# sunkafei/coffeedb

Measured on AMD Instinct MI355X. Metric: sa_build_GiB_per_s, higher is better.
Workload: dtype u64

## Files before the change

### coffeedb_amd/csrc/capi.hip

```cpp
#include <dirent.h>

#include <algorithm>
#include <chrono>
#include <condition_variable>
#include <cstdlib>
#include <cstring>
#include <thread>

#include "../../include/coffeedb_gpu.h"
#include "index_impl.h"

using namespace cdb;

namespace {

double wall_ms() {
    using namespace std::chrono;
    return duration<double, std::milli>(steady_clock::now().time_since_epoch()).count();
}

void set_error(Index& ix, const char* msg) {
    std::lock_guard<std::mutex> g(ix.err_mu);
    ix.err = msg;
}
// ... 1553 lines not shown
    else if (!std::strcmp(name, "pack_sa")) ix.pack_sa = value != 0;
    else if (!std::strcmp(name, "key_cost_model")) ix.key_cost_model = value != 0;
    else if (!std::strcmp(name, "gen_prebased")) ix.gen_prebased = value != 0;
    else if (!std::strcmp(name, "pack_entries")) ix.pack_entries = value != 0;
    else if (!std::strcmp(name, "segmented_sort")) ix.segmented_sort = value != 0;
    else if (!std::strcmp(name, "fold_root")) ix.fold_root = value != 0;
    else if (!std::strcmp(name, "fold_depth1")) ix.fold_depth1 = value != 0;
    else if (!std::strcmp(name, "flags_in_last_pass")) ix.flags_in_last_pass = value != 0;
    else if (!std::strcmp(name, "search_lanes")) ix.search_lanes = (value == 1 || value == 8) ? (int)value : 0;
    else if (!std::strcmp(name, "digit_bits")) ix.digit_bits = (int)value;
    else if (!std::strcmp(name, "fuse_keygen")) ix.fuse_keygen = value != 0;
    else if (!std::strcmp(name, "force_big_path")) ix.force_big_path = value != 0;
    else if (!std::strcmp(name, "debug_fail_build")) ix.debug_fail_build = value != 0;
    else if (!std::strcmp(name, "debug_no_segcap")) ix.debug_no_segcap = value != 0;
    else if (!std::strcmp(name, "debug_starve_group")) ix.debug_starve_group = (int)value;
    else if (!std::strcmp(name, "self_check")) ix.self_check = value < 0 ? 0 : value > 3 ? 3 : (int)value;
    else if (!std::strcmp(name, "premap_generation")) ix.premap_generation = value != 0;
    else if (!std::strcmp(name, "proof_cancel")) {
        if (value) proof_stop(ix);
    }
    else if (!std::strcmp(name, "debug_damage_after_build")) ix.debug_damage_after_build = value < 0 ? 0 : (uint64_t)value;
    else if (!std::strcmp(name, "debug_fail_self_check")) ix.debug_fail_self_check = value != 0;
    else if (!std::strcmp(name, "plain_tile_order")) ix.rws.plain_order = value != 0;
    else if (!std::strcmp(name, "key_coding")) ix.key_coding = (int)value;
    else if (!std::strcmp(name, "narrow_keys")) ix.narrow_keys = value != 0;
    else if (!std::strcmp(name, "single_query")) ix.use_single_query = value != 0;
    else if (!std::strcmp(name, "resident_query")) {
        std::lock_guard<std::mutex> g(ix.mu);
        if (value != 1) query_resident_stop(ix);
        ix.resident_mode = value <= 0 ? 0 : value == 1 ? 1 : 2;
        ix.resident_query = ix.resident_mode == 1;
        ix.single_streak = 0;
    }
    else if (!std::strcmp(name, "bucket_group_limit")) ix.bucket_group_limit = (uint64_t)value;
    else if (!std::strcmp(name, "query_hit_budget"))
        ix.query_hit_budget = value > 0 ? std::min<uint64_t>((uint64_t)value, 1ull << 31) : 1;
    else if (!std::strcmp(name, "coalesce_queries")) ix.coalesce_queries = value != 0;
    else if (!std::strcmp(name, "fast_search")) ix.use_fast_search = value != 0;
    else if (!std::strcmp(name, "wave_rows")) ix.use_wave_rows = value != 0;
    else if (!std::strcmp(name, "keep_keys")) ix.keep_keys = value != 0;
    else {
        set_error(ix, (std::string("unknown option: ") + name).c_str());
        return CDB_E_INVALID;
    }
    return CDB_OK;
}

int cdb_get_stat(const cdb_index* h, const char* name, double* value) {
    if (!h || !name || !value) return CDB_E_INVALID;
    const BuildStats& b = h->ix.bstats;
    const QueryStats& q = h->ix.qstats;
    struct { const char* n; double v; } tab[] = {
        {"build_ms", b.build_ms}, {"alloc_ms", b.alloc_ms}, {"free_ms", b.free_ms}, {"rounds", (double)b.rounds}, {"ext_rounds", (double)b.ext_rounds},
        {"dbl_rounds", (double)b.dbl_rounds}, {"unresolved_after_initial", (double)b.unresolved_initial},
        {"unresolved_max", (double)b.unresolved_max}, {"sort_passes", (double)b.sort_passes},
        {"sort_passes_skipped", (double)b.sort_passes_skipped}, {"isa_built", (double)b.isa_built}, {"fused_keygen", (double)b.fused_keygen}, {"dense_keys", (double)b.dense_keys}, {"key_layout", (double)b.key_layout}, {"bucketed", (double)b.bucketed}, {"bucket_groups", (double)b.bucket_groups}, {"segmented", (double)b.segmented}, {"fused_records", (double)b.fused_records}, {"sweep_records", (double)b.sweep_records}, {"vl_key_bits", (double)b.vl_key_bits}, {"partial_levels", (double)b.partial_levels}, {"list_rounds", (double)b.list_rounds}, {"pairclass_fused", (double)b.pairclass_fused}, {"group_sorts", (double)b.group_sorts}, {"group_sort_fallbacks", (double)b.group_sort_fallbacks}, {"vl_avg_len", b.vl_avg_len}, {"vl_rate", b.vl_rate}, {"vl_est_unresolved", b.vl_est_unresolved}, {"fixed_est_unresolved", b.fixed_est_unresolved}, {"gen_prebased", (double)b.gen_prebased}, {"root_folded", (double)b.root_folded}, {"flags_in_last_pass", (double)b.flags_in_last_pass}, {"msd_first", (double)b.msd_first}, {"bucket_low_digits", (double)b.bucket_low_digits}, {"key_directory_cells", h->ix.h_keydir.empty() ? 0.0 : (double)(h->ix.h_keydir.size() - 1)}, {"group_fallbacks", (double)h->ix.group_fallbacks}, {"dense_key_retries", (double)h->ix.dense_key_retries}, {"self_check_fallbacks", (double)h->ix.self_check_fallbacks}, {"sa_packed", h->ix.sa_packed ? 1.0 : 0.0}, {"sa_bytes_per_entry", h->ix.sa_packed ? 5.0 : (double)h->ix.width}, {"self_check_pairs", (double)h->ix.self_check_pairs}, {"self_check_ms", h->ix.self_check_ms}, {"self_check_coverage", h->ix.size > 1 ? (double)h->ix.self_check_pairs / (double)(h->ix.size - 1) : 0.0},
        {"order_proved", (h->ix.proof.state.load() == 2 || h->ix.proof.state.load() == 3 || (h->ix.self_check == 2 && h->ix.width != 0)) ? 1.0 : 0.0},
        {"proof_state", (double)h->ix.proof.state.load()}, {"proof_ms", h->ix.proof.ms}, {"proof_repair_ms", h->ix.proof.repair_ms},
        {"proof_pairs", (double)h->ix.proof.pairs}, {"proof_bad_pairs", (double)h->ix.proof.found[0]}, {"proof_invalid_entries", (double)h->ix.proof.found[1]}, {"proof_skipped_pairs", (double)h->ix.proof.skipped}, {"proof_mixed_pairs", (double)h->ix.proof.mixed},
        {"proof_runs", (double)h->ix.proof.runs}, {"pool_big_mallocs", (double)DevPool::get().big_mallocs()}, {"premap_ms", h->ix.proof.premap_ms}, {"premap_bytes", (double)h->ix.proof.premap_bytes},
        {"key_symbols", (double)b.key_symbols}, {"symbol_bits", (double)b.symbol_bits},
        {"alphabet", (double)b.alphabet}, {"digit_bits", (double)b.digit_bits}, {"final_depth", (double)b.final_depth}, {"compat_rotations", (double)b.compat_rotations},
        {"compat_depth", (double)b.compat_depth},
        {"host_upload_ms", h->ix.host_upload_ms}, {"host_free_ms", h->ix.host_free_ms},
        {"resident_answers", (double)h->ix.res_answers}, {"launched_answers", (double)h->ix.launched_answers}, {"resident_mode", (double)h->ix.resident_mode},
        {"query_ms", q.query_ms}, {"query_upload_ms", q.upload_ms}, {"query_device_ms", q.device_ms}, {"query_download_ms", q.download_ms}, {"query_hits", (double)q.nhits}, {"query_rows", (double)q.nrows},
    };
    for (auto& e : tab)
        if (!std::strcmp(e.n, name)) {
            *value = e.v;
            return CDB_OK;
        }
    return CDB_E_INVALID;
}

int cdb_profile_get(cdb_index* h, const char* kernel, double* total_ms, uint64_t* launches, uint64_t* bytes) {
    if (!h || !kernel) return CDB_E_INVALID;
    std::lock_guard<std::mutex> g(h->ix.mu);
    auto it = h->ix.prof.recs.find(kernel);
    if (it == h->ix.prof.recs.end()) return CDB_E_INVALID;
    if (total_ms) *total_ms = it->second.ms;
    if (launches) *launches = it->second.launches;
    if (bytes) *bytes = it->second.bytes;
    return CDB_OK;
}

int cdb_profile_dump(cdb_index* h, char* buf, size_t cap) {
    if (!h || !buf || cap == 0) return CDB_E_INVALID;
    std::lock_guard<std::mutex> g(h->ix.mu);
// ... 172 lines not shown
```

### coffeedb_amd/csrc/index_impl.h

```cpp
#pragma once
#include <atomic>
#include <condition_variable>
#include <mutex>
#include <thread>
#include <string>
#include <vector>

#include "common.h"
#include "radix_sort.h"

namespace cdb {

constexpr int TEXT_PAD = 128;

struct BuildStats {
    double build_ms = 0, alloc_ms = 0, free_ms = 0;
    int rounds = 0;
    int ext_rounds = 0;
    int dbl_rounds = 0;
    uint64_t unresolved_initial = 0;
    uint64_t unresolved_max = 0;
    int sort_passes = 0;
    int sort_passes_skipped = 0;
    int isa_built = 0;
    int fused_keygen = 0;
    int key_layout = 0;
    int dense_keys = 0;
    int bucketed = 0;
    int bucket_low_digits = 0;
    int bucket_groups = 0;
    int root_folded = 0;
    int flags_in_last_pass = 0;
    int msd_first = 0;
    int gen_prebased = 0;
    int fused_records = 0;
    int sweep_records = 0;
    int pairclass_fused = 0;
    int list_rounds = 0;
    int group_sorts = 0, group_sort_fallbacks = 0;
    int partial_levels = 0;
    int vl_key_bits = 0;
    double vl_avg_len = 0, vl_rate = 0, vl_est_unresolved = 0, fixed_est_unresolved = 0;
    int segmented = 0;
    uint64_t gather_items = 0;
    int key_symbols = 0, symbol_bits = 0, alphabet = 0, digit_bits = 8;
    uint64_t final_depth = 0;
    uint64_t compat_rotations = 0, compat_depth = 0;
};

struct QueryStats {
    double query_ms = 0;
    double upload_ms = 0, device_ms = 0, download_ms = 0;
    uint64_t nhits = 0, nrows = 0;
};

struct SingleKeys {
    const uint64_t* keys64 = nullptr;
    const uint32_t* keys32 = nullptr;
    const void* keylow = nullptr;
    int low_bits = 0, low_bytes = 0, nsym = 0;
    bool decisive = false;
    uint64_t klo = 0, khi = 0;
    bool ranged = false;
    uint64_t lo0 = 0, hi0 = 0;
};

struct Sa40 {
    const uint32_t* __restrict__ lo;
    const uint8_t* __restrict__ hi;
    __device__ __forceinline__ uint64_t operator[](uint64_t i) const { return (uint64_t)lo[i] | ((uint64_t)hi[i] << 32); }
};
struct Packed40 {};
template <typename T> struct SaOf {
    using val = T;
    using ptr = const T* __restrict__;
};
// ... 106 lines not shown

    RadixWorkspace rws;
    MsdWorkspace msd_ws;
    DevBuf scan_partials;
    uint64_t q_spec_cap = 0;
    DevBuf q_spec;
    DevBuf q_pat, q_offs, q_left, q_right, q_hoff, q_keys0, q_keys1, q_flags, q_rowptr, q_ids, q_counts, q_hitptr, q_hitoff;

    bool reference_compat = true;
    bool force_doubling = false;
    int initial_passes = 0;
    int key_symbols = 0;
    int sort_variant = 0;
    int search_lanes = 0;
    bool flags_in_last_pass = true;
    bool fold_depth1 = true;
    bool fold_root = true;
    bool segmented_sort = true;
    bool fuse_records = true;
    bool fuse_pairclass = true;
    bool list_rounds = true;
    int group_sort_cap = 4096;
    bool group_sort = true;
    bool partial_symbol = true;
    int vl_keys = 2;
    bool vl_off_once = false;
    bool sweep_records = true;
    bool pack_entries = true;
    bool msd_first = true;
    bool msd_pair = true;
    bool keyhist3 = true;
    int dense_key_retries = 0;
    int group_fallbacks = 0;
    uint64_t bucket_group_limit = 0;
    uint64_t self_check_pairs = 0;
    double self_check_ms = 0;
    int self_check = 3;
    int self_check_fallbacks = 0;
    bool debug_fail_self_check = false;
    struct Proof {
        std::thread th;
        std::atomic<int> state{0};
        std::atomic<bool> cancel{false};
        hipStream_t stream = nullptr;
        void* d_out = nullptr;
        double ms = 0, repair_ms = 0;
        uint64_t pairs = 0;
        uint64_t found[2] = {0, 0};
        uint64_t skipped = 0;
        uint64_t mixed = 0;
        uint64_t runs = 0;
        bool of_loaded_file = false;
        std::atomic<bool> busy{false};
        bool want_proof = false;
        double premap_ms = 0;
        uint64_t premap_bytes = 0;
    } proof;
    bool premap_generation = false;
    bool proof_in_repair = false;
    uint64_t debug_damage_after_build = 0;
    bool debug_no_segcap = false;
    int debug_starve_group = 0;
    bool debug_fail_build = false;
    bool force_big_path = false;
    bool fuse_keygen = true;
    int digit_bits = 0;
// ... 91 lines not shown
```

### coffeedb_amd/csrc/radix_sort.h

```cpp
#pragma once
#include <cstdlib>

#include "common.h"

namespace cdb {

constexpr int RS_MAX_PASSES = 16;

constexpr uint64_t RS_VAL_MASK = (1ull << 54) - 1;
constexpr uint32_t RS_SPIN_LIMIT_GROUPED = 1u << 18;
constexpr uint32_t RS_SPIN_LIMIT_PLAIN = 1u << 22;
constexpr int RS_GROUP = 8;

struct NoVal {};

template <typename K, typename V> struct RsTraits { static constexpr int IPT = 12; };
template <> struct RsTraits<uint64_t, uint32_t> { static constexpr int IPT = 15; };
template <> struct RsTraits<uint64_t, uint64_t> { static constexpr int IPT = 12; };

template <typename K>
__global__ __launch_bounds__(256) void rs_hist_kernel(const K* __restrict__ keys, uint64_t n, int begin_bit,
                                                      int npass, int dbits, uint32_t last_mask,
                                                      unsigned long long* __restrict__ ghist) {
    __shared__ uint32_t sh[RS_MAX_PASSES * 256];
// ... 1188 lines not shown
        if (need > status.bytes) {
            status.alloc(need + need / 4);
            CDB_HIP(hipMemsetAsync(status.p, 0, status.bytes, s));
            CDB_HIP(hipMemsetAsync(tickets.p, 0, 256 * sizeof(uint32_t), s));
            CDB_HIP(hipMemsetAsync(tickets.as<uint32_t>() + 260, 0, 256 * 8 * sizeof(uint32_t), s));
            epoch = 0;
        }
    }
    uint32_t next_epoch(hipStream_t s) {
        if (epoch == 255) {
            CDB_HIP(hipMemsetAsync(status.p, 0, status.bytes, s));
            CDB_HIP(hipMemsetAsync(tickets.p, 0, 256 * sizeof(uint32_t), s));
            CDB_HIP(hipMemsetAsync(tickets.as<uint32_t>() + 260, 0, 256 * 8 * sizeof(uint32_t), s));
            epoch = 0;
        }
        return ++epoch;
    }
    uint32_t* ticket_ptr(uint32_t e) { return tickets.as<uint32_t>() + (e & 255u); }
    uint32_t* xticket_ptr(uint32_t e) { return tickets.as<uint32_t>() + 260 + (e & 255u) * 8; }
    uint32_t* err_ptr() { return tickets.as<uint32_t>() + 256; }
    void release() { hist.release(); status.release(); tickets.release(); tile_doc.release(); seg1.release(); epoch = 0; }
};

template <typename K, typename V> inline const char* rs_kernel_name();
template <> inline const char* rs_kernel_name<uint64_t, uint32_t>() { return "rs_onesweep_k64_v32"; }
template <> inline const char* rs_kernel_name<uint64_t, uint64_t>() { return "rs_onesweep_k64_v64"; }
template <> inline const char* rs_kernel_name<uint64_t, NoVal>() { return "rs_onesweep_k64"; }
template <> inline const char* rs_kernel_name<uint32_t, uint32_t>() { return "rs_onesweep_k32_v32"; }
template <> inline const char* rs_kernel_name<uint32_t, uint64_t>() { return "rs_onesweep_k32_v64"; }
template <> inline const char* rs_kernel_name<uint32_t, NoVal>() { return "rs_onesweep_k32"; }

struct SortStats {
    int passes_run = 0, passes_skipped = 0;
};

inline bool rs_variant_has_gen(int v) {
    return v == 0 || v == 21 || v == 26 || v == 1 || v == 31 || v == 33 || v == 36 || v == 32;
}

struct SortPlan {
    int npass, begin_bit;
    uint32_t last_mask;
    std::vector<uint64_t> h_hist;
};

template <typename K, typename V, typename Cfg, typename Gen = NoGen, typename W = NoVal>
int radix_sort_cfg(hipStream_t s, RadixWorkspace& ws, Profiler& prof, K* k0, K* k1, V* v0, V* v1, uint64_t n,
                   int begin_bit, int end_bit, SortStats* stats, int dbits, const uint64_t* h_hist_in = nullptr,
                   const Gen* gen = nullptr, W* w0 = nullptr, W* w1 = nullptr, int lead_in = 0,
                   const unsigned long long* d_hist_in = nullptr, const SegFinalKeepArgs* keep = nullptr) {
    constexpr int IPT = Cfg::IPT;
    constexpr int TILE = Cfg::NT * IPT;
    constexpr bool HAS_V = !std::is_same<V, NoVal>::value;
    constexpr bool HAS_W = !std::is_same<W, NoVal>::value;
    constexpr bool GEN = !std::is_same<Gen, NoGen>::value;
    if (dbits < 1 || dbits > 8) dbits = 8;
    int lead = 0;
    if constexpr (GEN && HAS_W) lead = gen->low_bits / dbits;
    else if constexpr (HAS_W) lead = lead_in;
    if (HAS_W && !GEN && !h_hist_in && !d_hist_in) throw Error("radix_sort: split records need caller-supplied histograms (internal)");
    const int LEAD = lead;
    if (n == 0 || end_bit < begin_bit || (!LEAD && end_bit == begin_bit)) return 0;
    const int nbits = end_bit - begin_bit;
    const int kpass = (int)ceil_div(nbits, dbits);
    const int npass = kpass + LEAD;
    if (npass > RS_MAX_PASSES) throw Error("radix_sort: too many passes requested");
// ... 300 lines not shown
        const unsigned long long* dstart = d_starts + (size_t)p * 256;
        uint32_t* tk = grouped ? ws.xticket_ptr(e) : ws.ticket_ptr(e);
        int t = prof.begin(s);
#define CDB_SEG_LAUNCH(CFG, SEGT, SEGV)                                                                                       \
    hipLaunchKernelGGL((rs_onesweep_kernel<uint32_t, uint32_t, CFG, NoGen, W, SEGT>), dim3(grid), dim3(1024), 0, s,            \
                       (const uint32_t*)kb[cur], kb[cur ^ 1], (const uint32_t*)vb[cur], vb[cur ^ 1], m, shift, dmask, dstart, \
                       ws.status.as<uint64_t>(), tk, e, ws.err_ptr(), NoGen(), (const W*)wb[cur], wb[cur ^ 1], aux_shift,     \
                       SEGV)
        if (p == npass - 1) {
            if (grouped) CDB_SEG_LAUNCH(CfgG, SegFinalArgs, fin);
            else CDB_SEG_LAUNCH(CfgP, SegFinalArgs, fin);
            prof.end(t, (std::string("rs_seg_final") + wn + "_t16384").c_str(), m * (rec + (fin.elo ? 6 : 9)), s);
        } else {
            if (grouped) CDB_SEG_LAUNCH(CfgG, SegArgs, sa);
            else CDB_SEG_LAUNCH(CfgP, SegArgs, sa);
            prof.end(t, (std::string("rs_seg_k32_v32") + wn + "_t16384").c_str(), 2 * m * rec, s);
        }
#undef CDB_SEG_LAUNCH
        cur ^= 1;
        if (stats) stats->passes_run++;
    }
    int t = prof.begin(s);
    hipLaunchKernelGGL(rs_seg_edge_fix_kernel, dim3(tiles), dim3(256), 0, s, (const SegEdge*)fin.edges, d_tile_seg, d_segs, tiles,
                       fin.flags, fin.kbase, fin.kmagic, (unsigned long long*)nullptr, 1u, (const uint32_t*)ws.err_ptr());
    prof.end(t, "rs_seg_edge_fix", (uint64_t)tiles * 256 * sizeof(SegEdge), s);
    CDB_HIP(hipGetLastError());
}

constexpr int RS_MSD_HIST_TILES = 32;

template <typename W>
__global__ __launch_bounds__(1024) void rs_seg_hist_kernel(const uint32_t* __restrict__ keys, const W* __restrict__ aux, int lead, int npass,
                                                           const uint32_t* __restrict__ tile_seg, const SegInfo* __restrict__ segs,
                                                           uint32_t tiles, unsigned long long* __restrict__ hist) {
    constexpr int NC = 4, HC = 8 * 256 + 64 / NC;
    __shared__ uint32_t sh4[NC * HC];
    const int tid = threadIdx.x;
    uint32_t* const sh = sh4 + (tid & (NC - 1)) * HC;
    const uint32_t t0 = blockIdx.x * RS_MSD_HIST_TILES;
    const uint32_t t1 = t0 + RS_MSD_HIST_TILES < tiles ? t0 + RS_MSD_HIST_TILES : tiles;
    uint32_t cur = ~0u;
    auto flush = [&]() {
        __syncthreads();
        if (cur != ~0u)
            for (int i = tid; i < npass * 256; i += 1024) {
                uint32_t c = 0;
#pragma unroll
                for (int q = 0; q < NC; ++q) c += sh4[q * HC + i];
                if (c) atomicAdd(&hist[((size_t)cur * 8 + i / 256) * 256 + i % 256], (unsigned long long)c);
            }
        __syncthreads();
        for (int i = tid; i < NC * HC; i += 1024) sh4[i] = 0;
        __syncthreads();
    };
    for (uint32_t t = t0; t < t1; ++t) {
        const uint32_t g = tile_seg[t];
        if (g != cur) {
            flush();
            cur = g;
        }
        const SegInfo si = segs[g];
        const uint64_t base = si.begin + (uint64_t)(t - si.tile_begin) * RS_SEG_TILE;
        const uint32_t valid = (uint32_t)((si.end - base) < (uint64_t)RS_SEG_TILE ? (si.end - base) : (uint64_t)RS_SEG_TILE);
        auto count = [&](uint32_t k, uint32_t a) {
#pragma unroll
            for (int p = 0; p < 8; ++p) {
                if (p < npass) {
                    const uint32_t dg = p < lead ? (a >> (8 * p)) & 0xFFu : (k >> (8 * (p - lead))) & 0xFFu;
                    atomicAdd(&sh[p * 256 + dg], 1u);
                }
            }
        };
        const uint64_t end = base + valid;
        const uint64_t a0 = (base + 3) & ~3ull;
        const uint64_t q0 = a0 < end ? a0 : end;
        const uint32_t nquad = (uint32_t)((end - q0) / 4);
        if ((uint64_t)tid < q0 - base) count(keys[base + tid], lead > 0 ? (uint32_t)aux[base + tid] : 0u);
        {
            const uint64_t tb = q0 + 4ull * nquad;
            if ((uint64_t)tid < end - tb) count(keys[tb + tid], lead > 0 ? (uint32_t)aux[tb + tid] : 0u);
        }
        constexpr int QPT = RS_SEG_TILE / 4 / 1024;
        uint4 kq[QPT];
        uint32_t aq[QPT][4];
#pragma unroll
        for (int r = 0; r < QPT; ++r) {
            const uint32_t g = (uint32_t)r * 1024u + (uint32_t)tid;
            kq[r] = make_uint4(0, 0, 0, 0);
            aq[r][0] = aq[r][1] = aq[r][2] = aq[r][3] = 0;
            if (g < nquad) {
                kq[r] = *reinterpret_cast<const uint4*>(keys + q0 + 4ull * g);
                if (lead > 0) {
                    if constexpr (sizeof(W) == 4) {
                        const uint4 w = *reinterpret_cast<const uint4*>(aux + q0 + 4ull * g);
                        aq[r][0] = w.x; aq[r][1] = w.y; aq[r][2] = w.z; aq[r][3] = w.w;
                    } else if constexpr (sizeof(W) == 2) {
                        const uint2 w = *reinterpret_cast<const uint2*>(aux + q0 + 4ull * g);
                        aq[r][0] = w.x & 0xFFFFu; aq[r][1] = w.x >> 16; aq[r][2] = w.y & 0xFFFFu; aq[r][3] = w.y >> 16;
                    } else {
                        const uint32_t w = *reinterpret_cast<const uint32_t*>(aux + q0 + 4ull * g);
                        aq[r][0] = w & 0xFFu; aq[r][1] = (w >> 8) & 0xFFu; aq[r][2] = (w >> 16) & 0xFFu; aq[r][3] = w >> 24;
                    }
                }
            }
        }
#pragma unroll
        for (int r = 0; r < QPT; ++r) {
            const uint32_t g = (uint32_t)r * 1024u + (uint32_t)tid;
            if (g < nquad) {
                count(kq[r].x, aq[r][0]);
                count(kq[r].y, aq[r][1]);
                count(kq[r].z, aq[r][2]);
                count(kq[r].w, aq[r][3]);
            }
        }
    }
    flush();
}

constexpr int RS_GEN8_TILE = 8192;
constexpr uint32_t RS_TB_ROWS = 256;
static __global__ __launch_bounds__(256) void rs_tilecol_sum_kernel(const uint32_t* __restrict__ counts, uint32_t rows, const uint16_t* __restrict__ src_col,
                                                                    unsigned long long* __restrict__ partial) {
    const uint32_t d = threadIdx.x, b = blockIdx.x;
    const uint32_t c = src_col ? (uint32_t)src_col[d] : d;
    const uint32_t r0 = b * RS_TB_ROWS, r1 = r0 + RS_TB_ROWS < rows ? r0 + RS_TB_ROWS : rows;
    unsigned long long sum = 0;
    if (c < 256u)
        for (uint32_t r = r0; r < r1; ++r) sum += counts[(size_t)r * 256 + c];
    partial[(size_t)b * 256 + d] = sum;
}
static __global__ __launch_bounds__(1024) void rs_tilecol_total_kernel(const unsigned long long* __restrict__ partial, uint32_t blocks,
                                                                       unsigned long long* __restrict__ totals) {
    __shared__ unsigned long long s_q[4][256];
    const uint32_t d = threadIdx.x & 255u, g = threadIdx.x >> 8;
    const uint32_t per = (blocks + 3u) / 4u;
    const uint32_t b0 = g * per, b1 = b0 + per < blocks ? b0 + per : blocks;
    unsigned long long sum = 0;
    uint32_t b = b0;
    for (; b + 8 <= b1; b += 8) {
        unsigned long long v[8];
#pragma unroll
        for (int i = 0; i < 8; ++i) v[i] = partial[(size_t)(b + i) * 256 + d];
#pragma unroll
        for (int i = 0; i < 8; ++i) sum += v[i];
    }
    for (; b < b1; ++b) sum += partial[(size_t)b * 256 + d];
    s_q[g][d] = sum;
    __syncthreads();
    if (g == 0) totals[d] = s_q[0][d] + s_q[1][d] + s_q[2][d] + s_q[3][d];
// ... 308 lines not shown
```

### coffeedb_amd/csrc/sa_build.hip

```cpp
#include <algorithm>
#include <chrono>
#include <cmath>
#include <cstdlib>
#include <cstring>

#include "index_impl.h"
#include "records_sweep.h"
#include "vl_code.h"
#include "scan.h"

#ifndef RS_GATHER_ABL
#define RS_GATHER_ABL 0
#endif

namespace cdb {
namespace {

constexpr int KG_TILE = 2048;
constexpr int KG_LOOK = 64;

__global__ __launch_bounds__(256) void sa_bytecount_kernel(const uint8_t* __restrict__ text, uint64_t n,
                                                           unsigned long long* __restrict__ counts) {
    __shared__ uint32_t s[256];
    s[threadIdx.x] = 0;
// ... 2686 lines not shown
                        constexpr unsigned gather_wgs = 256u * 8u;
                        if (pack_seg)
                        hipLaunchKernelGGL((sa_bucket_records_lists_kernel<W, Packed40>), dim3(gather_wgs), dim3(256), 0, s,
                                           Sa40{E.as<uint32_t>(), sa_hi_buf.as<uint8_t>()},
                                           (const BucketItem*)d_items2.as<BucketItem>(), (const uint32_t*)list_len, tickets, text, n, doc_start,
                                           (const uint16_t*)d_symmap.as<uint16_t>(), (int)ix.bits, ix.mask, nsym, bbase, blow, bpass, g.gstart,
                                           g.b0, kbp[0], wb[0].as<W>(), ebp[0], d_bh2.as<unsigned long long>());
                        else
                        hipLaunchKernelGGL((sa_bucket_records_lists_kernel<W>), dim3(gather_wgs), dim3(256), 0, s, (const uint64_t*)E.as<uint64_t>(),
                                           (const BucketItem*)d_items2.as<BucketItem>(), (const uint32_t*)list_len, tickets, text, n, doc_start,
                                           (const uint16_t*)d_symmap.as<uint16_t>(), (int)ix.bits, ix.mask, nsym, bbase, blow, bpass, g.gstart,
                                           g.b0, kbp[0], wb[0].as<W>(), ebp[0], d_bh2.as<unsigned long long>());
                        ix.prof.end(t, "sa_bucket_records", g.elems * ((uint64_t)nsym + recb + sizeof(V)), s);
                        st.gather_items += g.elems / BR_ITEM;
                        hipLaunchKernelGGL(rs_seg_tilemap_kernel, dim3((unsigned)ceil_div(g.tiles, 256)), dim3(256), 0, s,
                                           (const SegInfo*)(d_segs.as<SegInfo>() + g.b0), gb, g.tiles, tile_seg.as<uint32_t>());
                        }
                        SegFinalArgs fin;
                        if (pack_seg) {
                            fin.elo = E.as<uint32_t>() + g.gstart;
                            fin.ehi = sa_hi_buf.as<uint8_t>() + g.gstart;
                        } else if (packed_out) {
                            fin.elo = kbp[dead] + g.gstart;
                            fin.ehi = sa_hi_buf.as<uint8_t>() + g.gstart;
                        } else {
                            fin.eout = (fuse_rec ? kb[dead].as<uint64_t>() : E.as<uint64_t>()) + g.gstart;
                        }
                        fin.flags = flags.as<uint8_t>() + g.gstart;
                        fin.edges = edges.as<SegEdge>();
                        fin.hi_shift = blow;
                        fin.low_bits = blow;
                        fin.kbase = fbase;
                        fin.kmagic = bmagic;
                        radix_sort_segmented<W>(s, ix.rws, ix.prof, kbp[0], kbp[1], ebp[0], ebp[1], wb[0].as<W>(), wb[1].as<W>(), g.elems,
                                                (const SegInfo*)(d_segs.as<SegInfo>() + g.b0), (const uint32_t*)tile_seg.as<uint32_t>(), gb,
                                                g.tiles, (const unsigned long long*)d_bh2.as<unsigned long long>(),
                                                d_starts.as<unsigned long long>(), bbits - blow, lowb, fin, &ss);
                        st.bucket_groups++;
                    }
                    CDB_HIP(hipStreamSynchronize(s));
                    if (sweep_rec || sweep_fused) ix.tbw.base.release();
                    if (fuse_rec) E = std::move(kb[dead]);
                    if (pack_seg) packed_out = true;
                    st.segmented = 1;
                }
            };
            if (seg_cap) {
                if (lowb == 0) run_segmented(uint8_t{});
                else if (lowb == 1) run_segmented(uint16_t{});
                else run_segmented(uint32_t{});
            } else {
            std::vector<uint64_t> bounds((size_t)nb * (nch + 1));
            CDB_HIP(hipMemcpyAsync(bounds.data(), d_bounds.p, bounds.size() * 8, hipMemcpyDeviceToHost, s));
            CDB_HIP(hipStreamSynchronize(s));
            const bool third = !packed && avail > (double)maxb * (2.0 * (keyb + lowb) + 2 * sizeof(V)) * 1.15;
            const double scratch = packed ? (double)maxb * recb
                                          : (double)maxb * (keyb + lowb + (third ? 2 : 1) * sizeof(V)) +
                                                (third ? (double)(n / 32) * (sizeof(I) + 16 + 2 * sizeof(V) + 1) : 0.0);
            uint64_t gcap = (uint64_t)std::max(0.0, (avail - scratch) * 0.85 / recb);
            if (ix.bucket_group_limit) gcap = std::min<uint64_t>(gcap, ix.bucket_group_limit);
            gcap = std::max<uint64_t>(std::min<uint64_t>(gcap, n), maxb);
            DevBuf k32g, lowg, k32t, lowt, ET, EX, elog, elot, d_bh, d_items;
            k32g.alloc(gcap * keyb);
            if (auxb) lowg.alloc(gcap * auxb);
            k32t.alloc(maxb * keyb);
            if (auxb) lowt.alloc(maxb * auxb);
// ... 394 lines not shown
                (void)scan_totals<uint64_t>(s, ix.scan_partials, hin, m, OpMax{}, (uint64_t)0);
                UpdateOut<SAW, I, R> uo{sval[rs].as<V>(), U.as<I>(), nh.as<uint8_t>(), m, doc_start, (int)ix.bits,
                                      ix.mask, hnew, sa, flags.as<uint8_t>(), rank.as<R>(), d_open.as<unsigned long long>(), order};
                scan_apply<uint64_t>(s, ix.scan_partials, hin, m, OpMax{}, (uint64_t)0, uo);
                st.dbl_rounds++;
            } else {
                hipLaunchKernelGGL((sa_update_kernel<SAW, I>), dim3((unsigned)ceil_div(m, 256)), dim3(256), 0, s,
                                   (const V*)sval[rs].as<V>(), (const I*)U.as<I>(), (const uint8_t*)nh.as<uint8_t>(), m,
                                   doc_start, (int)ix.bits, ix.mask, hnew, sa, flags.as<uint8_t>(), d_open.as<unsigned long long>(),
                                   vl_kb1 ? (const uint8_t*)hcov.as<uint8_t>() : nullptr, h_acc + (uint32_t)nsym2, lf.as<uint8_t>());
                h_acc += (uint32_t)nsym2;
                st.ext_rounds++;
                have_list = true;
                m_list = m;
                list_rs = rs;
            }
            ix.prof.end(t, "sa_update", m * (2 * sizeof(V) + sizeof(I) + 2 + (isa ? sizeof(R) : 0)), s);
        }
        h = hnew;
        st.rounds++;
        if (st.rounds > 80) throw Error("suffix-array refinement did not converge (internal error)");
    }
    };
    if constexpr (sizeof(V) == 8) {
        if (packed_out) refine(Sa40RW{sa_buf.as<uint32_t>(), sa_hi_buf.as<uint8_t>()});
        else refine(SaRW<V>{sa_buf.as<V>()});
    } else {
        refine(SaRW<V>{sa_buf.as<V>()});
    }
    if (ix.debug_fail_build) throw Error("debug: build failure requested (test hook)");
    if (ix.debug_starve_group == 1 && !ix.rws.plain_order) throw Error("radix sort look-back timed out (test hook)");
    st.final_depth = h;
    st.sort_passes = ss.passes_run;
    st.sort_passes_skipped = ss.passes_skipped;
    radix_check_error(s, ix.rws);
    CDB_HIP(hipStreamSynchronize(s));
    ix.sa_sorted = !(ix.reference_compat && high_bytes);
    ix.pivot_levels = 0;
    if (ix.key_nsym) {
        ix.d_symmap_q = std::move(d_symmap);
        std::memcpy(ix.h_symmap_q, h_map, sizeof(h_map));
    }
    if (ix.reference_compat && high_bytes) {
        if (!folded_roots.empty() && !depth1.empty()) {
            std::vector<CompatBucket> nodes;
            for (size_t b = 0; b < folded_roots.size(); ++b) {
                const CompatBucket r = folded_roots[b];
                if (depth1[b].done) {
                    const unsigned long long hs = r.lo + depth1[b].nend, ls = hs + depth1[b].nhigh;
                    if (depth1[b].nend) nodes.push_back(CompatBucket{r.lo, hs});
                    nodes.push_back(CompatBucket{hs, ls});
                    nodes.push_back(CompatBucket{ls, r.hi});
                } else {
                    nodes.push_back(r);
                }
            }
            folded_roots.swap(nodes);
        }
        const std::vector<CompatBucket>* roots = folded_roots.empty() ? nullptr : &folded_roots;
        auto reorder = [&](auto tag) {
            using T = decltype(tag);
            if (!apply_reference_order_oop<T>(ix, sa_buf, &sa_hi_buf, roots)) {
                apply_reference_order<T>(ix, sa_buf, &sa_hi_buf, roots);
                ix.drop_keys();
            }
        };
// ... 135 lines not shown
```

Before: 30.05.

## Add MSD segmented radix sort with shared-memory window finish

```diff
diff --git a/coffeedb_amd/csrc/capi.hip b/coffeedb_amd/csrc/capi.hip
--- a/coffeedb_amd/csrc/capi.hip
+++ b/coffeedb_amd/csrc/capi.hip
@@ -1609,6 +1609,8 @@
         ix.resident_query = ix.resident_mode == 1;
         ix.single_streak = 0;
     }
+    else if (!std::strcmp(name, "seg_msd")) ix.seg_msd = (value == 1 || value == 2) ? (int)value : 0;
+    else if (!std::strcmp(name, "msd_cap")) ix.msd_cap = value > 0 ? (uint32_t)std::min<int64_t>(value, RS_MSD_CAP) : 0;
     else if (!std::strcmp(name, "bucket_group_limit")) ix.bucket_group_limit = (uint64_t)value;
     else if (!std::strcmp(name, "query_hit_budget"))
         ix.query_hit_budget = value > 0 ? std::min<uint64_t>((uint64_t)value, 1ull << 31) : 1;
@@ -1631,7 +1633,7 @@
         {"build_ms", b.build_ms}, {"alloc_ms", b.alloc_ms}, {"free_ms", b.free_ms}, {"rounds", (double)b.rounds}, {"ext_rounds", (double)b.ext_rounds},
         {"dbl_rounds", (double)b.dbl_rounds}, {"unresolved_after_initial", (double)b.unresolved_initial},
         {"unresolved_max", (double)b.unresolved_max}, {"sort_passes", (double)b.sort_passes},
-        {"sort_passes_skipped", (double)b.sort_passes_skipped}, {"isa_built", (double)b.isa_built}, {"fused_keygen", (double)b.fused_keygen}, {"dense_keys", (double)b.dense_keys}, {"key_layout", (double)b.key_layout}, {"bucketed", (double)b.bucketed}, {"bucket_groups", (double)b.bucket_groups}, {"segmented", (double)b.segmented}, {"fused_records", (double)b.fused_records}, {"sweep_records", (double)b.sweep_records}, {"vl_key_bits", (double)b.vl_key_bits}, {"partial_levels", (double)b.partial_levels}, {"list_rounds", (double)b.list_rounds}, {"pairclass_fused", (double)b.pairclass_fused}, {"group_sorts", (double)b.group_sorts}, {"group_sort_fallbacks", (double)b.group_sort_fallbacks}, {"vl_avg_len", b.vl_avg_len}, {"vl_rate", b.vl_rate}, {"vl_est_unresolved", b.vl_est_unresolved}, {"fixed_est_unresolved", b.fixed_est_unresolved}, {"gen_prebased", (double)b.gen_prebased}, {"root_folded", (double)b.root_folded}, {"flags_in_last_pass", (double)b.flags_in_last_pass}, {"msd_first", (double)b.msd_first}, {"bucket_low_digits", (double)b.bucket_low_digits}, {"key_directory_cells", h->ix.h_keydir.empty() ? 0.0 : (double)(h->ix.h_keydir.size() - 1)}, {"group_fallbacks", (double)h->ix.group_fallbacks}, {"dense_key_retries", (double)h->ix.dense_key_retries}, {"self_check_fallbacks", (double)h->ix.self_check_fallbacks}, {"sa_packed", h->ix.sa_packed ? 1.0 : 0.0}, {"sa_bytes_per_entry", h->ix.sa_packed ? 5.0 : (double)h->ix.width}, {"self_check_pairs", (double)h->ix.self_check_pairs}, {"self_check_ms", h->ix.self_check_ms}, {"self_check_coverage", h->ix.size > 1 ? (double)h->ix.self_check_pairs / (double)(h->ix.size - 1) : 0.0},
+        {"sort_passes_skipped", (double)b.sort_passes_skipped}, {"isa_built", (double)b.isa_built}, {"fused_keygen", (double)b.fused_keygen}, {"dense_keys", (double)b.dense_keys}, {"key_layout", (double)b.key_layout}, {"bucketed", (double)b.bucketed}, {"bucket_groups", (double)b.bucket_groups}, {"segmented", (double)b.segmented}, {"msd_groups", (double)b.msd_groups}, {"msd_finished", (double)b.msd_finished}, {"msd_lsd_fallback", (double)b.msd_lsd_fallback}, {"msd_third_split", (double)b.msd_third_split}, {"fused_records", (double)b.fused_records}, {"sweep_records", (double)b.sweep_records}, {"vl_key_bits", (double)b.vl_key_bits}, {"partial_levels", (double)b.partial_levels}, {"list_rounds", (double)b.list_rounds}, {"pairclass_fused", (double)b.pairclass_fused}, {"group_sorts", (double)b.group_sorts}, {"group_sort_fallbacks", (double)b.group_sort_fallbacks}, {"vl_avg_len", b.vl_avg_len}, {"vl_rate", b.vl_rate}, {"vl_est_unresolved", b.vl_est_unresolved}, {"fixed_est_unresolved", b.fixed_est_unresolved}, {"gen_prebased", (double)b.gen_prebased}, {"root_folded", (double)b.root_folded}, {"flags_in_last_pass", (double)b.flags_in_last_pass}, {"msd_first", (double)b.msd_first}, {"bucket_low_digits", (double)b.bucket_low_digits}, {"key_directory_cells", h->ix.h_keydir.empty() ? 0.0 : (double)(h->ix.h_keydir.size() - 1)}, {"group_fallbacks", (double)h->ix.group_fallbacks}, {"dense_key_retries", (double)h->ix.dense_key_retries}, {"self_check_fallbacks", (double)h->ix.self_check_fallbacks}, {"sa_packed", h->ix.sa_packed ? 1.0 : 0.0}, {"sa_bytes_per_entry", h->ix.sa_packed ? 5.0 : (double)h->ix.width}, {"self_check_pairs", (double)h->ix.self_check_pairs}, {"self_check_ms", h->ix.self_check_ms}, {"self_check_coverage", h->ix.size > 1 ? (double)h->ix.self_check_pairs / (double)(h->ix.size - 1) : 0.0},
         {"order_proved", (h->ix.proof.state.load() == 2 || h->ix.proof.state.load() == 3 || (h->ix.self_check == 2 && h->ix.width != 0)) ? 1.0 : 0.0},
         {"proof_state", (double)h->ix.proof.state.load()}, {"proof_ms", h->ix.proof.ms}, {"proof_repair_ms", h->ix.proof.repair_ms},
         {"proof_pairs", (double)h->ix.proof.pairs}, {"proof_bad_pairs", (double)h->ix.proof.found[0]}, {"proof_invalid_entries", (double)h->ix.proof.found[1]}, {"proof_skipped_pairs", (double)h->ix.proof.skipped}, {"proof_mixed_pairs", (double)h->ix.proof.mixed},
diff --git a/coffeedb_amd/csrc/index_impl.h b/coffeedb_amd/csrc/index_impl.h
--- a/coffeedb_amd/csrc/index_impl.h
+++ b/coffeedb_amd/csrc/index_impl.h
@@ -42,6 +42,8 @@
     int vl_key_bits = 0;
     double vl_avg_len = 0, vl_rate = 0, vl_est_unresolved = 0, fixed_est_unresolved = 0;
     int segmented = 0;
+    int msd_groups = 0;
+    uint64_t msd_finished = 0, msd_lsd_fallback = 0, msd_third_split = 0;
     uint64_t gather_items = 0;
     int key_symbols = 0, symbol_bits = 0, alphabet = 0, digit_bits = 8;
     uint64_t final_depth = 0;
@@ -214,6 +216,8 @@
     bool keyhist3 = true;
     int dense_key_retries = 0;
     int group_fallbacks = 0;
+    int seg_msd = 0;
+    uint32_t msd_cap = 0;
     uint64_t bucket_group_limit = 0;
     uint64_t self_check_pairs = 0;
     double self_check_ms = 0;
diff --git a/coffeedb_amd/csrc/radix_sort.h b/coffeedb_amd/csrc/radix_sort.h
--- a/coffeedb_amd/csrc/radix_sort.h
+++ b/coffeedb_amd/csrc/radix_sort.h
@@ -1244,6 +1244,8 @@
 
 struct SortStats {
     int passes_run = 0, passes_skipped = 0;
+    uint64_t msd_finished = 0, msd_lsd_fallback = 0, msd_third_split = 0;
+    int msd_groups = 0;
 };
 
 inline bool rs_variant_has_gen(int v) {
@@ -1610,7 +1612,7 @@
 template <typename W>
 __global__ __launch_bounds__(1024) void rs_seg_hist_kernel(const uint32_t* __restrict__ keys, const W* __restrict__ aux, int lead, int npass,
                                                            const uint32_t* __restrict__ tile_seg, const SegInfo* __restrict__ segs,
-                                                           uint32_t tiles, unsigned long long* __restrict__ hist) {
+                                                           uint32_t tiles, unsigned long long* __restrict__ hist, int first = 0) {
     constexpr int NC = 4, HC = 8 * 256 + 64 / NC;
     __shared__ uint32_t sh4[NC * HC];
     const int tid = threadIdx.x;
@@ -1644,7 +1646,7 @@
 #pragma unroll
             for (int p = 0; p < 8; ++p) {
                 if (p < npass) {
-                    const uint32_t dg = p < lead ? (a >> (8 * p)) & 0xFFu : (k >> (8 * (p - lead))) & 0xFFu;
+                    const uint32_t dg = p < lead ? (a >> (8 * p)) & 0xFFu : (k >> (8 * (p - lead + first))) & 0xFFu;
                     atomicAdd(&sh[p * 256 + dg], 1u);
                 }
             }
@@ -1694,6 +1696,348 @@
         }
     }
     flush();
+}
+
+constexpr int RS_MSD_NT = 1024, RS_MSD_IPT = 16;
+constexpr uint32_t RS_MSD_CAP = RS_MSD_NT * RS_MSD_IPT;
+
+struct MsdWindow {
+    unsigned long long begin;
+    uint32_t len, top;
+};
+
+static __global__ __launch_bounds__(256) void rs_msd_plan_kernel(const unsigned long long* __restrict__ starts, const SegInfo* __restrict__ segs,
+                                                                 uint32_t nsub, uint32_t cap, MsdWindow* __restrict__ wins, uint32_t max_wins,
+                                                                 SegInfo* __restrict__ big, uint32_t max_big, unsigned long long* __restrict__ ctr) {
+    const uint32_t g = blockIdx.x * 256 + threadIdx.x;
+    if (g >= nsub) return;
+    const SegInfo si = segs[g];
+    const unsigned long long* st = starts + (size_t)g * 8 * 256;
+    unsigned long long wb = si.begin, fin = 0, bigr = 0;
+    uint32_t wlen = 0;
+    auto flush = [&]() {
+        if (!wlen) return;
+        const unsigned long long i = atomicAdd(ctr + 0, 1ull);
+        if (i < max_wins) wins[i] = MsdWindow{wb, wlen, si.top};
+        fin += wlen;
+        wlen = 0;
+    };
+    for (int d = 0; d < 256; ++d) {
+        const unsigned long long c0 = st[d], c1 = d < 255 ? st[d + 1] : si.end;
+        const unsigned long long len = c1 - c0;
+        if (!len) continue;
+        if (len > cap) {
+            flush();
+            const unsigned long long i = atomicAdd(ctr + 1, 1ull);
+            if (i < max_big) big[i] = SegInfo{c0, c1, 0u, 0u, 0ull, 0ull};
+            bigr += len;
+            continue;
+        }
+        if (wlen + len > cap) flush();
+        if (!wlen) wb = c0;
+        wlen += (uint32_t)len;
+    }
+    flush();
+    if (fin) atomicAdd(ctr + 2, fin);
+    if (bigr) atomicAdd(ctr + 3, bigr);
+}
+
+template <typename W>
+__global__ __launch_bounds__(RS_MSD_NT) void rs_msd_finish_kernel(const uint32_t* __restrict__ keys, const uint32_t* __restrict__ vals,
+                                                                  const W* __restrict__ aux, const MsdWindow* __restrict__ wins,
+                                                                  SegFinalArgs fin) {
+    constexpr int NT = RS_MSD_NT, IPT = RS_MSD_IPT, NW = NT / 64, WCHUNK = 64 * IPT;
+    __shared__ uint64_t s_stage[RS_MSD_CAP];
+    __shared__ uint32_t s_whist[NW][256];
+    __shared__ uint32_t s_tstart[256];
+    __shared__ uint32_t s_wsum[4];
+    const int tid = threadIdx.x, lane = tid & 63, wave = tid >> 6;
+    const MsdWindow w = wins[blockIdx.x];
+    const uint32_t valid = w.len;
+    const uint64_t base = w.begin;
+    const int lb = fin.low_bits;
+    const uint32_t lmask = (1u << lb) - 1u;
+    const int npass = (24 + lb) / 8;
+    const uint32_t wbase = wave * WCHUNK + lane;
+    const uint32_t* const kw = keys + base;
+    const uint32_t* const vw = vals + base;
+    const W* const aw = aux + base;
+    uint32_t key[IPT], lo[IPT], hi4[IPT / 4], rank[IPT];
+#pragma unroll
+    for (int j = 0; j < IPT / 4; ++j) hi4[j] = 0;
+#pragma unroll
+    for (int j = 0; j < IPT; ++j) {
+        const uint32_t li = wbase + j * 64;
+        key[j] = ~0u;
+        lo[j] = 0;
+        if (li < valid) {
+            const uint32_t a = (uint32_t)aw[li];
+            key[j] = ((kw[li] & 0xFFFFFFu) << lb) | (a & lmask);
+            lo[j] = vw[li];
+            hi4[j >> 2] |= ((a >> fin.hi_shift) & 0xFFu) << (8 * (j & 3));
+        }
+    }
+    uint8_t* const s_bytes = reinterpret_cast<uint8_t*>(s_stage);
+#pragma unroll 1
+    for (int p = 0; p < npass; ++p) {
+        const bool last = p == npass - 1;
+        const int sh = 8 * p;
+        for (int i = tid; i < NW * 256; i += NT) (&s_whist[0][0])[i] = 0;
+        __syncthreads();
+#pragma unroll
+        for (int j = 0; j < IPT; ++j) rank[j] = atomicAdd(&s_whist[wave][(key[j] >> sh) & 0xFFu], 1u);
+        __syncthreads();
+        uint32_t cnt = 0, incl = 0;
+        if (tid < 256) {
+#pragma unroll
+            for (int q = 0; q < NW; ++q) {
+                const uint32_t t = s_whist[q][tid];
+                s_whist[q][tid] = cnt;
+                cnt += t;
+            }
+            incl = cnt;
+#pragma unroll
+            for (int off = 1; off < 64; off <<= 1) {
+                const uint32_t v = __shfl_up(incl, off);
+                if (lane >= off) incl += v;
+            }
+            if (lane == 63) s_wsum[wave] = incl;
+        }
+        __syncthreads();
+        if (tid < 256) {
+            uint32_t wpre = 0;
+#pragma unroll
+            for (int q = 0; q < 4; ++q)
+                if (q < wave) wpre += s_wsum[q];
+            s_tstart[tid] = wpre + incl - cnt;
+        }
+        __syncthreads();
+#pragma unroll
+        for (int j = 0; j < IPT; ++j) {
+            const uint32_t d = (key[j] >> sh) & 0xFFu;
+            rank[j] += s_tstart[d] + s_whist[wave][d];
+            s_bytes[rank[j]] = (uint8_t)(hi4[j >> 2] >> (8 * (j & 3)));
+        }
+        __syncthreads();
+        const uint32_t r0 = last ? (uint32_t)tid : wbase;
+        const uint32_t rs = last ? (uint32_t)NT : 64u;
+#pragma unroll
+        for (int j = 0; j < IPT / 4; ++j) {
+            const uint32_t q = r0 + 4 * j * rs;
+            hi4[j] = (uint32_t)s_bytes[q] | ((uint32_t)s_bytes[q + rs] << 8) | ((uint32_t)s_bytes[q + 2 * rs] << 16) |
+                     ((uint32_t)s_bytes[q + 3 * rs] << 24);
+        }
+        __syncthreads();
+#pragma unroll
+        for (int j = 0; j < IPT; ++j) s_stage[rank[j]] = ((uint64_t)key[j] << 32) | lo[j];
+        __syncthreads();
+        if (!last) {
+#pragma unroll
+            for (int j = 0; j < IPT; ++j) {
+                const uint64_t v = s_stage[wbase + j * 64];
+                key[j] = (uint32_t)(v >> 32);
+                lo[j] = (uint32_t)v;
+            }
+            __syncthreads();
+        }
+    }
+    const uint64_t ktop = (uint64_t)w.top << (24 + lb);
+#pragma unroll
+    for (int j = 0; j < IPT; ++j) {
+        const uint32_t i = j * NT + tid;
+        if (i >= valid) continue;
+        const uint64_t v = s_stage[i];
+        const uint32_t k = (uint32_t)(v >> 32);
+        const bool head = i == 0 || (uint32_t)(s_stage[i - 1] >> 32) != k;
+        const bool tail = i + 1 >= valid || (uint32_t)(s_stage[i + 1] >> 32) != k;
+        uint32_t f = head ? 1u : 0u;
+        if (!(head && tail)) {
+            const uint64_t kc = ktop | (uint64_t)k;
+            const bool exhausted = fin.kmagic ? (kc - __umul64hi(kc, fin.kmagic) * fin.kbase) == 0
+                                              : (kc & (uint64_t)(fin.kbase - 1u)) == 0;
+            if (!exhausted) f |= 2u;
+        }
+        const uint64_t slot = base + i;
+        fin.flags[slot] = (uint8_t)f;
+        if (fin.elo) {
+            fin.elo[slot] = (uint32_t)v;
+            fin.ehi[slot] = (uint8_t)(hi4[j >> 2] >> (8 * (j & 3)));
+        } else {
+            fin.eout[slot] = ((uint64_t)((hi4[j >> 2] >> (8 * (j & 3))) & 0xFFu) << 32) | (uint64_t)(uint32_t)v;
+        }
+    }
+}
+
+inline bool rs_msd_eligible(const SegInfo* h_segs, uint32_t nseg, int key_bits, int lead, size_t wbytes) {
+    if (key_bits != 32 || lead > 1 || wbytes > 2) return false;
+    for (uint32_t g = 0; g < nseg; ++g)
+        if (h_segs[g].rot_b) return false;
+    return true;
+}
+
+template <typename W>
+bool radix_sort_segmented_msd(hipStream_t s, RadixWorkspace& ws, Profiler& prof, uint32_t* k0, uint32_t* k1, uint32_t* v0, uint32_t* v1,
+                              W* w0, W* w1, uint64_t m, const SegInfo* d_segs, const SegInfo* h_segs, uint32_t nseg, uint32_t tiles,
+                              const uint32_t* d_tile_seg, const unsigned long long* d_hist, unsigned long long* d_starts, int lead,
+                              SegFinalArgs fin, int mode,
+                              uint32_t cap, SortStats* stats) {
+    if (!rs_atomic_rank_ok(s)) return false;
+    if (cap == 0 || cap > RS_MSD_CAP) cap = RS_MSD_CAP;
+    const int p1 = lead + 3, p2 = lead + 2;
+    std::vector<unsigned long long> hh((size_t)nseg * 8 * 256);
+    CDB_HIP(hipMemcpyAsync(hh.data(), d_hist, hh.size() * sizeof(unsigned long long), hipMemcpyDeviceToHost, s));
+    CDB_HIP(hipStreamSynchronize(s));
+    if (mode != 2) {
+        double fit = 0;
+        std::vector<double> c2(256), pre(257);
+        for (uint32_t g = 0; g < nseg; ++g) {
+            const double size = (double)(h_segs[g].end - h_segs[g].begin);
+            if (size <= 0) continue;
+            for (int d = 0; d < 256; ++d) c2[d] = (double)hh[((size_t)g * 8 + p2) * 256 + d];
+            std::sort(c2.begin(), c2.end());
+            pre[0] = 0;
+            for (int d = 0; d < 256; ++d) pre[d + 1] = pre[d] + c2[d];
+            for (int d = 0; d < 256; ++d) {
+                const double c1 = (double)hh[((size_t)g * 8 + p1) * 256 + d];
+                if (c1 <= 0) continue;
+                const double lim = (double)cap * size / c1;
+                const int q = (int)(std::upper_bound(c2.begin(), c2.end(), lim) - c2.begin());
+                fit += c1 * pre[q] / size;
+            }
+        }
+        const double f = m ? fit / (double)m : 0.0;
+        const double msd = 2.3 + 2.8 * f + (1.0 - f) * (lead + 2.3);
+        if (msd > (double)(lead + 4) - 0.3) return false;
+    }
+    const int npass0 = lead + 4;
+    hipLaunchKernelGGL(rs_seg_digit_start_kernel, dim3(nseg), dim3(256), 0, s, d_hist, d_segs, npass0, d_starts);
+    const bool grouped = ws.allow_group && !ws.plain_order;
+    using CfgG = RsCfg<16, true, true, 1024, false, 1, 0, 4, false, true, true, 1, RS_GROUP>;
+    using CfgP = RsCfg<16, true, true, 1024, false, 1, 0, 4, false, true>;
+    const char* wn = sizeof(W) == 1 ? "_w8" : "_w16";
+    const size_t rec = 8 + sizeof(W);
+    auto split = [&](int from, int byte, const SegArgs& sa, const unsigned long long* dstart) {
+        ws.prepare((uint64_t)sa.tiles * RS_SEG_TILE, RS_SEG_TILE, s);
+        const uint32_t e = ws.next_epoch(s);
+        uint32_t* tk = grouped ? ws.xticket_ptr(e) : ws.ticket_ptr(e);
+        const uint32_t grid = grouped ? (uint32_t)(ceil_div(sa.tiles, 8u * RS_GROUP) * 8u * RS_GROUP) : sa.tiles;
+        uint32_t* kb[2] = {k0, k1};
+        uint32_t* vb[2] = {v0, v1};
+        W* wb[2] = {w0, w1};
+        int t = prof.begin(s);
+#define CDB_MSD_SPLIT(CFG)                                                                                                            \
+    hipLaunchKernelGGL((rs_onesweep_kernel<uint32_t, uint32_t, CFG, NoGen, W, SegArgs>), dim3(grid), dim3(1024), 0, s,                \
+                       (const uint32_t*)kb[from], kb[from ^ 1], (const uint32_t*)vb[from], vb[from ^ 1], m, 8 * byte, 0xFFu, dstart,  \
+                       ws.status.as<uint64_t>(), tk, e, ws.err_ptr(), NoGen(), (const W*)wb[from], wb[from ^ 1], -1, sa)
+        if (grouped) CDB_MSD_SPLIT(CfgG);
+        else CDB_MSD_SPLIT(CfgP);
+#undef CDB_MSD_SPLIT
+        prof.end(t, (std::string("rs_seg_msd_split") + wn + "_t16384").c_str(), 2 * m * rec, s);
+        if (stats) stats->passes_run++;
+    };
+    SegArgs sa1;
+    sa1.tile_seg = d_tile_seg;
+    sa1.segs = d_segs;
+    sa1.tiles = tiles;
+    sa1.start_stride = 8 * 256;
+    split(0, 3, sa1, d_starts + (size_t)p1 * 256);
+    std::vector<SegInfo> h2;
+    uint32_t tiles2 = 0;
+    for (uint32_t g = 0; g < nseg; ++g) {
+        unsigned long long b = h_segs[g].begin;
+        for (int d = 0; d < 256; ++d) {
+            const unsigned long long c = hh[((size_t)g * 8 + p1) * 256 + d];
+            if (!c) continue;
+            h2.push_back(SegInfo{b, b + c, tiles2, (uint32_t)d, 0ull, 0ull});
+            tiles2 += (uint32_t)ceil_div((uint64_t)c, (uint64_t)RS_SEG_TILE);
+            b += c;
+        }
+    }
+    const uint32_t nsub = (uint32_t)h2.size();
+    DevBuf d_segs2, d_tseg2, d_hist2, d_starts2, d_wins, d_big, d_ctr;
+    d_segs2.alloc((size_t)nsub * sizeof(SegInfo));
+    d_tseg2.alloc((size_t)tiles2 * sizeof(uint32_t));
+    d_hist2.alloc((size_t)nsub * 8 * 256 * sizeof(unsigned long long));
+    d_starts2.alloc((size_t)nsub * 8 * 256 * sizeof(unsigned long long));
+    const uint64_t max_wins = 3 * (m / cap) + nsub + 2, max_big = m / ((uint64_t)cap + 1) + 1;
+    d_wins.alloc((size_t)max_wins * sizeof(MsdWindow));
+    d_big.alloc((size_t)max_big * sizeof(SegInfo));
+    d_ctr.alloc(4 * sizeof(unsigned long long));
+    CDB_HIP(hipMemcpyAsync(d_segs2.p, h2.data(), (size_t)nsub * sizeof(SegInfo), hipMemcpyHostToDevice, s));
+    CDB_HIP(hipMemsetAsync(d_hist2.p, 0, d_hist2.bytes, s));
+    CDB_HIP(hipMemsetAsync(d_ctr.p, 0, d_ctr.bytes, s));
+    hipLaunchKernelGGL(rs_seg_tilemap_kernel, dim3((unsigned)ceil_div(tiles2, 256u)), dim3(256), 0, s, (const SegInfo*)d_segs2.as<SegInfo>(), nsub,
+                       tiles2, d_tseg2.as<uint32_t>());
+    int t = prof.begin(s);
+    hipLaunchKernelGGL((rs_seg_hist_kernel<W>), dim3((unsigned)ceil_div(tiles2, (uint32_t)RS_MSD_HIST_TILES)), dim3(1024), 0, s, (const uint32_t*)k1,
+                       (const W*)w1, 0, 1, (const uint32_t*)d_tseg2.as<uint32_t>(), (const SegInfo*)d_segs2.as<SegInfo>(), tiles2,
+                       d_hist2.as<unsigned long long>(), 2);
+    prof.end(t, "rs_seg_hist", m * 4, s);
+    hipLaunchKernelGGL(rs_seg_digit_start_kernel, dim3(nsub), dim3(256), 0, s, (const unsigned long long*)d_hist2.as<unsigned long long>(),
+                       (const SegInfo*)d_segs2.as<SegInfo>(), 1, d_starts2.as<unsigned long long>());
+    SegArgs sa2;
+    sa2.tile_seg = d_tseg2.as<uint32_t>();
+    sa2.segs = d_segs2.as<SegInfo>();
+    sa2.tiles = tiles2;
+    sa2.start_stride = 8 * 256;
+    split(1, 2, sa2, d_starts2.as<unsigned long long>());
+    t = prof.begin(s);
+    hipLaunchKernelGGL(rs_msd_plan_kernel, dim3((unsigned)ceil_div(nsub, 256u)), dim3(256), 0, s,
+                       (const unsigned long long*)d_starts2.as<unsigned long long>(), (const SegInfo*)d_segs2.as<SegInfo>(), nsub, cap,
+                       d_wins.as<MsdWindow>(), (uint32_t)max_wins, d_big.as<SegInfo>(), (uint32_t)max_big, d_ctr.as<unsigned long long>());
+    prof.end(t, "rs_msd_plan", (uint64_t)nsub * 256 * 8, s);
+    unsigned long long ctr[4];
+    CDB_HIP(hipMemcpyAsync(ctr, d_ctr.p, sizeof(ctr), hipMemcpyDeviceToHost, s));
+    CDB_HIP(hipStreamSynchronize(s));
+    if (ctr[0] > max_wins || ctr[1] > max_big || ctr[2] + ctr[3] != m) throw Error("radix_sort_segmented_msd: window plan overflow (internal)");
+    if (stats) {
+        stats->msd_finished += ctr[2];
+        stats->msd_lsd_fallback += ctr[3];
+        stats->msd_groups++;
+    }
+    if (ctr[0]) {
+        t = prof.begin(s);
+        hipLaunchKernelGGL((rs_msd_finish_kernel<W>), dim3((unsigned)ctr[0]), dim3(RS_MSD_NT), 0, s, (const uint32_t*)k0, (const uint32_t*)v0,
+                           (const W*)w0, (const MsdWindow*)d_wins.as<MsdWindow>(), fin);
+        prof.end(t, (std::string("rs_msd_finish") + wn).c_str(), ctr[2] * (rec + (fin.elo ? 6 : 9)), s);
+    }
+    if (ctr[1]) {
+        const uint32_t nbig = (uint32_t)ctr[1];
+        std::vector<SegInfo> hb(nbig);
+        CDB_HIP(hipMemcpyAsync(hb.data(), d_big.p, (size_t)nbig * sizeof(SegInfo), hipMemcpyDeviceToHost, s));
+        CDB_HIP(hipStreamSynchronize(s));
+        std::sort(hb.begin(), hb.end(), [](const SegInfo& a, const SegInfo& b) { return a.begin < b.begin; });
+        uint32_t tiles3 = 0;
+        for (SegInfo& c : hb) {
+            c.tile_begin = tiles3;
+            tiles3 += (uint32_t)ceil_div((uint64_t)(c.end - c.begin), (uint64_t)RS_SEG_TILE);
+        }
+        DevBuf d_segs3, d_tseg3, d_hist3, d_starts3, d_edges3;
+        d_segs3.alloc((size_t)nbig * sizeof(SegInfo));
+        d_tseg3.alloc((size_t)tiles3 * sizeof(uint32_t));
+        d_hist3.alloc((size_t)nbig * 8 * 256 * sizeof(unsigned long long));
+        d_starts3.alloc((size_t)nbig * 8 * 256 * sizeof(unsigned long long));
+        if (tiles3 > tiles) {
+            d_edges3.alloc((size_t)tiles3 * 256 * sizeof(SegEdge));
+            fin.edges = d_edges3.as<SegEdge>();
+        }
+        CDB_HIP(hipMemcpyAsync(d_segs3.p, hb.data(), (size_t)nbig * sizeof(SegInfo), hipMemcpyHostToDevice, s));
+        CDB_HIP(hipMemsetAsync(d_hist3.p, 0, d_hist3.bytes, s));
+        hipLaunchKernelGGL(rs_seg_tilemap_kernel, dim3((unsigned)ceil_div(tiles3, 256u)), dim3(256), 0, s, (const SegInfo*)d_segs3.as<SegInfo>(),
+                           nbig, tiles3, d_tseg3.as<uint32_t>());
+        t = prof.begin(s);
+        hipLaunchKernelGGL((rs_seg_hist_kernel<W>), dim3((unsigned)ceil_div(tiles3, (uint32_t)RS_MSD_HIST_TILES)), dim3(1024), 0, s,
+                           (const uint32_t*)k0, (const W*)w0, lead, lead + 2, (const uint32_t*)d_tseg3.as<uint32_t>(),
+                           (const SegInfo*)d_segs3.as<SegInfo>(), tiles3, d_hist3.as<unsigned long long>(), 0);
+        prof.end(t, "rs_seg_hist", ctr[3] * (4 + (lead > 0 ? sizeof(W) : 0)), s);
+        radix_sort_segmented<W>(s, ws, prof, k0, k1, v0, v1, w0, w1, m, (const SegInfo*)d_segs3.as<SegInfo>(), (const uint32_t*)d_tseg3.as<uint32_t>(),
+                                nbig, tiles3, (const unsigned long long*)d_hist3.as<unsigned long long>(), d_starts3.as<unsigned long long>(), 16,
+                                lead, fin, stats);
+        CDB_HIP(hipStreamSynchronize(s));
+    }
+    CDB_HIP(hipGetLastError());
+    CDB_HIP(hipStreamSynchronize(s));
+    return true;
 }
 
 constexpr int RS_GEN8_TILE = 8192;
diff --git a/coffeedb_amd/csrc/sa_build.hip b/coffeedb_amd/csrc/sa_build.hip
--- a/coffeedb_amd/csrc/sa_build.hip
+++ b/coffeedb_amd/csrc/sa_build.hip
@@ -2742,6 +2742,14 @@
                         fin.low_bits = blow;
                         fin.kbase = fbase;
                         fin.kmagic = bmagic;
+                        const bool msd_ok = ix.seg_msd != 1 && (!fuse_rec || packed_out) &&
+                                            rs_msd_eligible(h_segs.data() + g.b0, gb, bbits - blow, lowb, sizeof(W));
+                        if (!(msd_ok && radix_sort_segmented_msd<W>(s, ix.rws, ix.prof, kbp[0], kbp[1], ebp[0], ebp[1], wb[0].as<W>(),
+                                                                     wb[1].as<W>(), g.elems, (const SegInfo*)(d_segs.as<SegInfo>() + g.b0),
+                                                                     h_segs.data() + g.b0, gb, g.tiles, (const uint32_t*)tile_seg.as<uint32_t>(),
+                                                                     (const unsigned long long*)d_bh2.as<unsigned long long>(),
+                                                                     d_starts.as<unsigned long long>(), lowb, fin, ix.seg_msd,
+                                                                     ix.msd_cap, &ss)))
                         radix_sort_segmented<W>(s, ix.rws, ix.prof, kbp[0], kbp[1], ebp[0], ebp[1], wb[0].as<W>(), wb[1].as<W>(), g.elems,
                                                 (const SegInfo*)(d_segs.as<SegInfo>() + g.b0), (const uint32_t*)tile_seg.as<uint32_t>(), gb,
                                                 g.tiles, (const unsigned long long*)d_bh2.as<unsigned long long>(),
@@ -3202,6 +3210,10 @@
     if (ix.debug_starve_group == 1 && !ix.rws.plain_order) throw Error("radix sort look-back timed out (test hook)");
     st.final_depth = h;
     st.sort_passes = ss.passes_run;
+    st.msd_groups = ss.msd_groups;
+    st.msd_finished = ss.msd_finished;
+    st.msd_lsd_fallback = ss.msd_lsd_fallback;
+    st.msd_third_split = ss.msd_third_split;
     st.sort_passes_skipped = ss.passes_skipped;
     radix_check_error(s, ix.rws);
     CDB_HIP(hipStreamSynchronize(s));
```

Result: no change. 29.85 (median of 3 runs) (-0.7%).
